# mkocabas/EpipolarPose

Measured on NVIDIA H100. Metric: multi-view samples/sec (4-view 256x256, bs32), higher is better.
Workload: dtype f16x3 (fp32 operands split into two fp16 planes, 3-pass error-compensated wgmma f16, f32 accumulate: fp32-grade results)

## Files before the change

### epipolarpose_b200/csrc/common.cuh

```cuda
#pragma once
#include <cuda_runtime.h>
#include <stdint.h>
#include <stdio.h>
#include <stdarg.h>
#include "../../include/epb.h"

void epb_set_error(const char* fmt, ...);

#define EPB_CHECK_ARG(cond)                                                   \
  do {                                                                        \
    if (!(cond)) {                                                            \
      epb_set_error("%s:%d: invalid argument: %s", __FILE__, __LINE__, #cond); \
      return EPB_EINVAL;                                                      \
    }                                                                         \
  } while (0)

#define EPB_CUDA(call)                                                        \
  do {                                                                        \
    cudaError_t e__ = (call);                                                 \
    if (e__ != cudaSuccess) {                                                 \
      epb_set_error("%s:%d: %s -> %s", __FILE__, __LINE__, #call,             \
                    cudaGetErrorString(e__));                                 \
      return EPB_ECUDA;                                                       \
    }                                                                         \
  } while (0)

#define EPB_LAUNCH_CHECK() EPB_CUDA(cudaGetLastError())

enum { EPB_WS_SOFTARGMAX = 1, EPB_WS_HMLOSS = 2, EPB_WS_BNCOEF = 3, EPB_WS_WPLANES = 4,
       EPB_WS_FPAIR = 5, EPB_WS_BNPART = 6, EPB_WS_SABWD = 7, EPB_WS_PATCHINV = 8, EPB_WS_KMEANS = 9 };
int epb_workspace(int kind, size_t bytes, cudaStream_t st, void** out);

static inline cudaStream_t as_stream(epb_stream_t s) { return (cudaStream_t)s; }

constexpr int kNumSMs = 132;

__device__ __forceinline__ float warp_sum(float v) {
#pragma unroll
  for (int o = 16; o > 0; o >>= 1) v += __shfl_xor_sync(0xffffffffu, v, o);
  return v;
}
__device__ __forceinline__ double warp_sum(double v) {
#pragma unroll
  for (int o = 16; o > 0; o >>= 1) v += __shfl_xor_sync(0xffffffffu, v, o);
  return v;
}
__device__ __forceinline__ float warp_max(float v) {
#pragma unroll
  for (int o = 16; o > 0; o >>= 1) v = fmaxf(v, __shfl_xor_sync(0xffffffffu, v, o));
  return v;
}
__device__ __forceinline__ float4 ldg_stream(const float4* p) {
  float4 r;
  asm volatile("ld.global.nc.L1::no_allocate.v4.f32 {%0,%1,%2,%3}, [%4];"
               : "=f"(r.x), "=f"(r.y), "=f"(r.z), "=f"(r.w) : "l"(p));
  return r;
}
```

### epipolarpose_b200/csrc/conv16.cu

```cuda
#include "split16_common.cuh"

namespace {

constexpr int BM = 128;
constexpr int kThreads16 = 384;
constexpr int kConsumers = 256;
constexpr int kStageBudget = 200 * 1024;
constexpr int kBoxBytes = 16 * 128;

struct Plan16 {
  epb_phase_grid grid;
  int Cout;
  int Wv, Hv;
  int T, CB;
  int n_tiles;
  int accumulate;
  int m_fastest;
  int splits;
  int koff[EPB_MAX_TAPS];
};

struct Maps16 {
  CUtensorMap a[4];
  CUtensorMap w;
  CUtensorMap out;
};

template <int BN>
struct Cfg16 {
  static constexpr int A_PLANE = BM * 128;
  static constexpr int B_PLANE = BN * 128;
  static constexpr int A_BYTES = 2 * A_PLANE;
  static constexpr int B_BYTES = 2 * B_PLANE;
  static constexpr int STAGE = A_BYTES + B_BYTES;
  static constexpr int S_ = kStageBudget / STAGE;
  static constexpr int S = S_ > 6 ? 6 : S_;
  static constexpr int BOX_BYTES = (kConsumers / 32) * kBoxBytes;
  static constexpr int STAT_BYTES = (kConsumers / 32) * 2 * BN * 4;
  static constexpr int SMEM =
      S * STAGE + BOX_BYTES + 1024  + 256  + STAT_BYTES;
  static_assert(SMEM <= 227 * 1024, "shared memory budget");
  static_assert(S >= 2, "ring too shallow");
};

template <int BN, bool SPLIT>
__global__ void __launch_bounds__(kThreads16, 1)
conv16_kernel(const __grid_constant__ Plan16 P, const __grid_constant__ Maps16 maps,
              const float* __restrict__ in_sc, const float* __restrict__ w_sc,
              const float* __restrict__ bias, double* __restrict__ stats) {
  using C = Cfg16<BN>;
  const epb_phase_grid& G = P.grid;
  constexpr int BOXES = C::S * C::STAGE;
  constexpr int CTRL = BOXES + C::BOX_BYTES;
  extern __shared__ uint8_t smem_raw[];
  tc::Ring<C::S, C::STAGE> ring(smem_raw, 0, CTRL, CTRL + 64);
  float* sstat = reinterpret_cast<float*>(ring.sm + CTRL + 256);

  const int warp = threadIdx.x >> 5, lane = threadIdx.x & 31;
  const int KB = P.T * P.CB;
  const int total_tiles = G.tiles * P.n_tiles;
  const int items = SPLIT ? total_tiles * P.splits : total_tiles;
  auto tile_of = [&](int item) { return SPLIT ? item % total_tiles : item; };
  auto kb_lo = [&](int s) { return SPLIT ? (int)((int64_t)s * KB / P.splits) : (s ? KB : 0); };
  auto nt_of = [&](int tile) { return P.m_fastest ? tile / G.tiles : tile % P.n_tiles; };
  auto mt_of = [&](int tile) { return P.m_fastest ? tile % G.tiles : tile / P.n_tiles; };

  if (threadIdx.x == 0) ring.init(1, kConsumers / 32);
  __syncthreads();

  if (warp < 4) {
    if (warp == 0 && lane == 0) {
      for (int v = 0; v < 4; ++v) tc::tma_prefetch_desc(&maps.a[v]);
      tc::tma_prefetch_desc(&maps.w);
      tc::tma_prefetch_desc(&maps.out);
      for (int item = blockIdx.x; item < items; item += gridDim.x) {
        const int tile = tile_of(item), s = SPLIT ? item / total_tiles : 0;
        const int nt = nt_of(tile);
        int w0, h0, n0;
        G.tile_origin(mt_of(tile), w0, h0, n0);
        const int kb0 = kb_lo(s), kb1 = kb_lo(s + 1);
        int t = kb0 / P.CB, cb = kb0 % P.CB;
        for (int kb = kb0; kb < kb1; ++kb) {
          tc::mbar_wait(ring.empty(ring.stage), ring.phase ^ 1);
          const uint32_t fb = ring.full(ring.stage);
          tc::mbar_arrive_expect_tx(fb, C::STAGE);
          const uint32_t a_dst = ring.stage_addr(ring.stage);
          const CUtensorMap* am = &maps.a[G.map[t]];
          const int cx = cb * 64, wx = w0 + G.dwq[t], hx = h0 + G.dhq[t];
          tc::tma_load_5d(a_dst, am, fb, cx, wx, hx, n0, 0);
          tc::tma_load_5d(a_dst + C::A_PLANE, am, fb, cx, wx, hx, n0, 1);
          const uint32_t b_dst = a_dst + C::A_BYTES;
          const int kx = P.koff[t] + cx, rx = nt * BN;
          tc::tma_load_3d(b_dst, &maps.w, fb, kx, rx, 0);
          tc::tma_load_3d(b_dst + C::B_PLANE, &maps.w, fb, kx, rx, 1);
          if (++cb == P.CB) { cb = 0; ++t; }
          ring.advance();
        }
      }
    }
    return;
  }

  const int wgc = (warp >> 2) - 1;
  const int ct = threadIdx.x - 128;
  float* wstat = sstat + (ct >> 5) * 2 * BN;
  const int lc = (lane & 3) * 2;
  const int rb = wgc * 64 + (warp & 3) * 16;
  const int ra = rb + (lane >> 2);
  uint8_t* box = ring.sm + BOXES + (ct >> 5) * kBoxBytes;
  const uint32_t box_addr = tc::smem_u32(box);
  auto chunk = [&](int jj) { return ((2 * jj + ((lane & 3) >> 1)) ^ (lane >> 2)) * 16 + (lane & 1) * 8; };
  const float alpha = in_sc[1] * w_sc[1];
  const int twh = G.tw * G.th;
  if (stats) {
    for (int c = ct; c < (kConsumers / 32) * 2 * BN; c += kConsumers) sstat[c] = 0.f;
    tc::named_sync(1, kConsumers);
  }

  float acc[BN / 2];
  int nt_prev = -1;
  for (int item = blockIdx.x; item < items; item += gridDim.x) {
    const int tile = tile_of(item), s = SPLIT ? item / total_tiles : 0;
    const int nt = nt_of(tile);
    if (stats && nt_prev >= 0 && nt != nt_prev)
      tc::stats_flush<BN, kConsumers / 32>(sstat, ct, nt_prev, P.Cout, stats);
    nt_prev = nt;
#pragma unroll
    for (int i = 0; i < BN / 2; ++i) acc[i] = 0.f;
    for (int kb = kb_lo(s), kb1 = kb_lo(s + 1); kb < kb1; ++kb)
      ring.consume(acc, [&](uint32_t st) {
        const uint32_t a_hi = st + wgc * 64 * 128, b_hi = st + C::A_BYTES;
#pragma unroll
        for (int kk = 0; kk < 4; ++kk)
          tc::mma3_f16<0, 0>(acc, tc::desc_kmajor_sw128(a_hi + kk * 32),
                             tc::desc_kmajor_sw128(a_hi + C::A_PLANE + kk * 32),
                             tc::desc_kmajor_sw128(b_hi + kk * 32),
                             tc::desc_kmajor_sw128(b_hi + C::B_PLANE + kk * 32));
      });
    ring.drain(acc);

    int w0, h0, n0;
    G.tile_origin(mt_of(tile), w0, h0, n0);
    bool srow[2];
#pragma unroll
    for (int h = 0; h < 2; ++h) {
      const int r = ra + 8 * h;
      const int w = w0 + r % G.tw, hh = h0 + (r / G.tw) % G.th, n = n0 + r / twh;
      srow[h] = w < G.Wp && hh < G.Hp && n < G.N;
    }
    const int bx = w0 + rb % G.tw, by = h0 + (rb / G.tw) % G.th, bz = n0 + rb / twh;
    const bool band = SPLIT || (bx < P.Wv && by < P.Hv && bz < G.N);
#pragma unroll
    for (int q = 0; q < BN / 32; ++q) {
      if (lane == 0) tc::tma_store_wait_read<0>();
      __syncwarp();
#pragma unroll
      float v[4][2][2];
#pragma unroll
      for (int jj = 0; jj < 4; ++jj) {
        const int col = nt * BN + 32 * q + 8 * jj + lc;
        float2 b = make_float2(0.f, 0.f);
        if (bias && col < P.Cout) b = *reinterpret_cast<const float2*>(bias + col);
#pragma unroll
        for (int h = 0; h < 2; ++h) {
          v[jj][h][0] = acc[16 * q + 4 * jj + 2 * h] * alpha + b.x;
          v[jj][h][1] = acc[16 * q + 4 * jj + 2 * h + 1] * alpha + b.y;
          *reinterpret_cast<float2*>(box + 128 * ((lane >> 2) + 8 * h) + chunk(jj)) =
              make_float2(v[jj][h][0], v[jj][h][1]);
        }
      }
      tc::fence_proxy_async();
      __syncwarp();
      const int c0 = nt * BN + 32 * q;
      if (lane == 0 && band && c0 < P.Cout) {
        if constexpr (SPLIT) tc::tma_store_4d(&maps.out, box_addr, c0, 0, (mt_of(tile) * BM + rb) / 16, s);
        else if (P.accumulate) tc::tma_reduce_add_4d(&maps.out, box_addr, c0, bx, by, bz);
        else tc::tma_store_4d(&maps.out, box_addr, c0, bx, by, bz);
        tc::tma_store_commit();
      }
      if (stats) {
#pragma unroll
        for (int jj = 0; jj < 4; ++jj) tc::stats_add<BN>(wstat, 32 * q + 8 * jj + lc, v[jj], srow);
      }
    }
  }
  if (stats && nt_prev >= 0) tc::stats_flush<BN, kConsumers / 32>(sstat, ct, nt_prev, P.Cout, stats);
  if (lane == 0) tc::tma_store_wait<0>();
}

struct Reduce16 {
  epb_phase_grid grid;
  int Cout, Wv, Hv, splits;
  int64_t sw, sh, sn;
};

__global__ void __launch_bounds__(256)
conv16_splitk_reduce(const __grid_constant__ Reduce16 R, const float* __restrict__ ws,
                     const float* __restrict__ bias, float* __restrict__ out,
                     double* __restrict__ stats) {
  __shared__ double red[2][8][128];
  const epb_phase_grid& G = R.grid;
  const int tx = threadIdx.x, ty = threadIdx.y;
  const int c = (blockIdx.x * 32 + tx) * 4;
  const bool cok = c < R.Cout;
  const int64_t M = (int64_t)G.N * G.Hp * G.Wp;
  const int64_t split_stride = (int64_t)G.tiles * BM * R.Cout;
  float b[4] = {0.f, 0.f, 0.f, 0.f};
  if (bias && cok)
    for (int e = 0; e < 4; ++e) b[e] = bias[c + e];
  double s1[4] = {0.0, 0.0, 0.0, 0.0}, s2[4] = {0.0, 0.0, 0.0, 0.0};
  if (cok) {
    for (int64_t m = (int64_t)blockIdx.y * 8 + ty; m < M; m += (int64_t)gridDim.y * 8) {
      const int w = (int)(m % G.Wp);
      const int64_t q = m / G.Wp;
      const int h = (int)(q % G.Hp), n = (int)(q / G.Hp);
      const int mt = w / G.tw + G.tiles_w * (h / G.th + G.tiles_h * (n / G.tn));
      const int r = w % G.tw + G.tw * (h % G.th + G.th * (n % G.tn));
      const float* src = ws + ((int64_t)mt * BM + r) * R.Cout + c;
      float4 v = *reinterpret_cast<const float4*>(src);
      for (int s = 1; s < R.splits; ++s) {
        const float4 u = *reinterpret_cast<const float4*>(src + s * split_stride);
        v.x += u.x; v.y += u.y; v.z += u.z; v.w += u.w;
      }
      v.x += b[0]; v.y += b[1]; v.z += b[2]; v.w += b[3];
      if (w < R.Wv && h < R.Hv)
        *reinterpret_cast<float4*>(out + n * R.sn + h * R.sh + w * R.sw + c) = v;
      const float a[4] = {v.x, v.y, v.z, v.w};
      for (int e = 0; e < 4; ++e) {
        s1[e] += a[e];
        s2[e] += (double)a[e] * a[e];
      }
    }
  }
  if (!stats) return;
  for (int e = 0; e < 4; ++e) {
    red[0][ty][tx * 4 + e] = s1[e];
    red[1][ty][tx * 4 + e] = s2[e];
  }
  __syncthreads();
  if (ty == 0 && cok)
    for (int e = 0; e < 4; ++e) {
      double t1 = 0.0, t2 = 0.0;
      for (int y = 0; y < 8; ++y) {
        t1 += red[0][y][tx * 4 + e];
        t2 += red[1][y][tx * 4 + e];
      }
      atomicAdd(stats + c + e, t1);
      atomicAdd(stats + R.Cout + c + e, t2);
    }
}

inline int conv16_bn(int Cout) { return Cout <= 64 ? 64 : 128; }

constexpr int kSplitMinKB = 4;
constexpr int kSplitLongKB = 16;

int conv16_run(const epb_conv_geom* g, const epb_half* in, const float* in_sc, const epb_half* w,
               const float* w_sc, const float* bias, float* out, double* stats, int splits,
               float* ws, epb_stream_t stream) {
  int rc = epb_conv_geom_check(g);
  if (rc) return rc;
  EPB_CHECK_ARG(in && in_sc && w && w_sc && out);
  EPB_CHECK_ARG(g->Cin % 64 == 0 && g->Cout % 4 == 0 && g->Cout >= 4);
  EPB_CHECK_ARG(g->is == 1 || g->is == 2);
  EPB_CHECK_ARG(!(stats && g->accumulate));
  EPB_CHECK_ARG((reinterpret_cast<uintptr_t>(in) & 127) == 0 && (reinterpret_cast<uintptr_t>(w) & 15) == 0);
  EPB_CHECK_ARG((reinterpret_cast<uintptr_t>(out) & 15) == 0 && (reinterpret_cast<uintptr_t>(bias) & 7) == 0);
  Plan16 P;
  Maps16 maps;
  memset(&maps, 0, sizeof(maps));
  bool dense;
  rc = epb_plan_phase_grid(g, in, BM, P.grid, maps.a, dense);
  if (rc) return rc;
  const int64_t Ho = dense ? 1 : g->Ho, Wo = dense ? P.grid.Wp : g->Wo, os = dense ? 1 : g->os;
  const int64_t ph = dense ? 0 : g->ph, pw = dense ? 0 : g->pw;
  P.Cout = g->Cout;
  P.Wv = dense ? P.grid.Wp : (g->Wo - g->pw + g->os - 1) / g->os;
  P.Hv = dense ? 1 : (g->Ho - g->ph + g->os - 1) / g->os;
  P.T = g->T; P.CB = g->Cin / 64; P.accumulate = g->accumulate;
  P.splits = splits;
  float* const view = out + (ph * Wo + pw) * g->Cout;
  if (splits == 1) {
    const int bw = P.grid.tw < 16 ? P.grid.tw : 16;
    const int bh = P.grid.th < 16 / bw ? P.grid.th : 16 / bw;
    const int64_t C4 = (int64_t)g->Cout * 4;
    const cuuint64_t dims[4] = {(cuuint64_t)g->Cout, (cuuint64_t)P.Wv, (cuuint64_t)P.Hv,
                                (cuuint64_t)P.grid.N};
    const cuuint64_t strides[3] = {(cuuint64_t)(os * C4), (cuuint64_t)(os * Wo * C4),
                                   (cuuint64_t)(Ho * Wo * C4)};
    const cuuint32_t box[4] = {32, (cuuint32_t)bw, (cuuint32_t)bh, (cuuint32_t)(16 / (bw * bh))};
    rc = epb_encode_map(&maps.out, CU_TENSOR_MAP_DATA_TYPE_FLOAT32, 4, view, dims, strides, box,
                        CU_TENSOR_MAP_L2_PROMOTION_NONE, "output");
    if (rc) return rc;
  } else {
    const int64_t C4 = (int64_t)g->Cout * 4;
    const cuuint64_t dims[4] = {(cuuint64_t)g->Cout, 16, (cuuint64_t)P.grid.tiles * (BM / 16),
                                (cuuint64_t)splits};
    const cuuint64_t strides[3] = {(cuuint64_t)C4, (cuuint64_t)(16 * C4),
                                   (cuuint64_t)((int64_t)P.grid.tiles * BM * C4)};
    const cuuint32_t box[4] = {32, 16, 1, 1};
    rc = epb_encode_map(&maps.out, CU_TENSOR_MAP_DATA_TYPE_FLOAT32, 4, ws, dims, strides, box,
                        CU_TENSOR_MAP_L2_PROMOTION_NONE, "split-K workspace");
    if (rc) return rc;
  }
  for (int t = 0; t < g->T; ++t) P.koff[t] = g->wt[t] * g->Cin;
  P.m_fastest = stats != nullptr;
  const int bn = conv16_bn(g->Cout);
  P.n_tiles = (g->Cout + bn - 1) / bn;
  const int64_t K = (int64_t)g->Tw * g->Cin;
  const cuuint64_t dims[3] = {(cuuint64_t)K, (cuuint64_t)g->Cout, 2};
  const cuuint64_t strides[2] = {(cuuint64_t)K * 2, (cuuint64_t)K * 2 * g->Cout};
  const cuuint32_t box[3] = {64, (cuuint32_t)bn, 1};
  rc = epb_encode_map(&maps.w, CU_TENSOR_MAP_DATA_TYPE_FLOAT16, 3, w, dims, strides, box,
                      CU_TENSOR_MAP_L2_PROMOTION_L2_256B, "weights");
  if (rc) return rc;
  const int64_t tiles = (int64_t)P.grid.tiles * P.n_tiles;
  cudaStream_t st = as_stream(stream);
  if (splits == 1) {
    const unsigned grid = (unsigned)(tiles < kNumSMs ? tiles : kNumSMs);
    if (bn == 64)
      return tc::launch<conv16_kernel<64, false>>(grid, kThreads16, Cfg16<64>::SMEM, st, P, maps,
                                                  in_sc, w_sc, bias, stats);
    return tc::launch<conv16_kernel<128, false>>(grid, kThreads16, Cfg16<128>::SMEM, st, P, maps,
                                                 in_sc, w_sc, bias, stats);
  }
  P.m_fastest = 0;
  const int64_t items = tiles * splits;
  const unsigned grid = (unsigned)(items < kNumSMs ? items : kNumSMs);
  const float* no_bias = nullptr;
  double* no_stats = nullptr;
  rc = bn == 64 ? tc::launch<conv16_kernel<64, true>>(grid, kThreads16, Cfg16<64>::SMEM, st, P, maps,
                                                      in_sc, w_sc, no_bias, no_stats)
                : tc::launch<conv16_kernel<128, true>>(grid, kThreads16, Cfg16<128>::SMEM, st, P,
                                                       maps, in_sc, w_sc, no_bias, no_stats);
  if (rc) return rc;
  Reduce16 R;
  R.grid = P.grid;
  R.Cout = g->Cout; R.Wv = P.Wv; R.Hv = P.Hv; R.splits = splits;
  R.sw = os * g->Cout; R.sh = os * Wo * g->Cout; R.sn = Ho * Wo * g->Cout;
  const int64_t M = (int64_t)P.grid.N * P.grid.Hp * P.grid.Wp;
  const unsigned gx = (unsigned)((g->Cout + 127) / 128);
  int64_t gy = (M + 7) / 8, cap = 4 * kNumSMs / gx + 1;
  if (gy > cap) gy = cap;
  conv16_splitk_reduce<<<dim3(gx, (unsigned)gy), dim3(32, 8), 0, st>>>(R, ws, bias, view, stats);
  EPB_LAUNCH_CHECK();
  return EPB_OK;
}

}

extern "C" __attribute__((visibility("default"))) int epb_conv16_fprop(
    const epb_conv_geom* g, const epb_half* in, const float* in_sc, const epb_half* w,
    const float* w_sc, const float* bias, float* out, double* stats, epb_stream_t stream) {
  return conv16_run(g, in, in_sc, w, w_sc, bias, out, stats, 1, nullptr, stream);
}

extern "C" __attribute__((visibility("default"))) int epb_conv16_splits(const epb_conv_geom* g,
                                                                          int* splits,
                                                                          long long* ws_floats) {
  int rc = epb_conv_geom_check(g);
  if (rc) return rc;
  EPB_CHECK_ARG(splits && ws_floats && g->Cin % 64 == 0 && g->Cout >= 4);
  epb_phase_grid G;
  bool dense;
  rc = epb_tile_phase_grid(g, BM, G, dense);
  if (rc) return rc;
  const int bn = conv16_bn(g->Cout);
  const int64_t tiles = (int64_t)G.tiles * ((g->Cout + bn - 1) / bn);
  const int64_t kb = (int64_t)g->T * (g->Cin / 64);
  int64_t s = kNumSMs / tiles;
  if (s > kb / kSplitMinKB) s = kb / kSplitMinKB;
  if (s < 4 && kb < kSplitLongKB * s) s = 1;
  if (s < 1) s = 1;
  *splits = (int)s;
  *ws_floats = s > 1 ? s * G.tiles * BM * g->Cout : 0;
  return EPB_OK;
}

extern "C" __attribute__((visibility("default"))) int epb_conv16_fprop_splitk(
    const epb_conv_geom* g, const epb_half* in, const float* in_sc, const epb_half* w,
    const float* w_sc, const float* bias, float* out, double* stats, int splits, float* ws,
    long long ws_floats, epb_stream_t stream) {
  int rc = epb_conv_geom_check(g);
  if (rc) return rc;
  EPB_CHECK_ARG(!g->accumulate);
  EPB_CHECK_ARG(g->Cin % 64 == 0 && splits >= 1 && splits <= g->T * (g->Cin / 64));
  if (splits > 1) {
    epb_phase_grid G;
    bool dense;
    rc = epb_tile_phase_grid(g, BM, G, dense);
    if (rc) return rc;
    EPB_CHECK_ARG(ws && (reinterpret_cast<uintptr_t>(ws) & 15) == 0);
    EPB_CHECK_ARG(ws_floats >= (long long)splits * G.tiles * BM * g->Cout);
  }
  return conv16_run(g, in, in_sc, w, w_sc, bias, out, stats, splits, ws, stream);
}
```

### epipolarpose_b200/csrc/split16.cu

```cuda
#include <cuda_fp16.h>
#include "common.cuh"

namespace {

constexpr int kThreads = 256;
constexpr float kHalfMax = 65504.f;

__device__ __forceinline__ void split2(float a, float b, float s, uint32_t& hi, uint32_t& lo) {
  a = fminf(fmaxf(a * s, -kHalfMax), kHalfMax);
  b = fminf(fmaxf(b * s, -kHalfMax), kHalfMax);
  const __half2 h = __floats2half2_rn(a, b);
  const float2 hf = __half22float2(h);
  const __half2 l = __floats2half2_rn(a - hf.x, b - hf.y);
  hi = *reinterpret_cast<const uint32_t*>(&h);
  lo = *reinterpret_cast<const uint32_t*>(&l);
}
__device__ __forceinline__ void split8(const float (&v)[8], float s, uint4& hi, uint4& lo) {
  split2(v[0], v[1], s, hi.x, lo.x);
  split2(v[2], v[3], s, hi.y, lo.y);
  split2(v[4], v[5], s, hi.z, lo.z);
  split2(v[6], v[7], s, hi.w, lo.w);
}
__device__ __forceinline__ float2 h2f(uint32_t u) {
  return __half22float2(*reinterpret_cast<const __half2*>(&u));
// ... 323 lines not shown
    sc[0] = s;
    sc[1] = 1.f / s;
  }
  for (int64_t i = (int64_t)blockIdx.x * kThreads + threadIdx.x; i < n4; i += (int64_t)gridDim.x * kThreads) {
    const float4 v = ldg_stream(src + i);
    uint2 hi, lo;
    split2(v.x, v.y, s, hi.x, lo.x);
    split2(v.z, v.w, s, hi.y, lo.y);
    dst[i] = hi;
    dst[n4 + i] = lo;
  }
}


struct RowMap {
  int C4, tpr, rpi, chunks;
};
inline RowMap make_rowmap(int C) {
  RowMap r;
  r.C4 = C / 4;
  r.tpr = r.C4 < kThreads ? r.C4 : kThreads;
  r.rpi = kThreads / r.tpr;
  if (r.rpi < 1) r.rpi = 1;
  r.chunks = (r.C4 + r.tpr - 1) / r.tpr;
  return r;
}

__device__ __forceinline__ float4 mask4(float4 dy, float4 xv, const uint2* mask_hi, int64_t i,
                                        float4 s, float4 b, int relu) {
  if (mask_hi) {
    const uint2 m = mask_hi[i];
    return make_float4((m.x & 0x7fffu) ? dy.x : 0.f, (m.x & 0x7fff0000u) ? dy.y : 0.f,
                       (m.y & 0x7fffu) ? dy.z : 0.f, (m.y & 0x7fff0000u) ? dy.w : 0.f);
  }
  if (relu) {
    return make_float4(fmaf(xv.x, s.x, b.x) > 0.f ? dy.x : 0.f, fmaf(xv.y, s.y, b.y) > 0.f ? dy.y : 0.f,
                       fmaf(xv.z, s.z, b.z) > 0.f ? dy.z : 0.f, fmaf(xv.w, s.w, b.w) > 0.f ? dy.w : 0.f);
  }
  return dy;
}

template <int MASK>
__device__ __forceinline__ uint2 load_mask(const uint2* mask, int64_t i) {
  if (MASK == 1) return __ldg(mask + i);
  const unsigned byte = __ldg(reinterpret_cast<const uint8_t*>(mask) + (i >> 1));
  return make_uint2((i & 1) ? (byte >> 4) : (byte & 15u), 0u);
}

template <int MASK>
__global__ void __launch_bounds__(kThreads, 3)
bn_bwd_partial_kernel(const float4* __restrict__ dy, const float4* __restrict__ x,
                      const uint2* __restrict__ mask_hi, const float4* __restrict__ scale,
                      const float4* __restrict__ shift, const float4* __restrict__ mean,
                      const float4* __restrict__ invstd, int relu, int64_t M, int C, RowMap rm,
                      float* __restrict__ parts, uint32_t* __restrict__ bound_bits) {
  if (bound_bits && blockIdx.x == 0 && blockIdx.y == 0 && threadIdx.x == 0) *bound_bits = 0u;
  const int slot = threadIdx.x / rm.tpr, tin = threadIdx.x % rm.tpr;
  const int c4 = blockIdx.y * rm.tpr + tin;
  const bool active = (c4 < rm.C4) && (slot < rm.rpi);
  const int64_t nblk = (M + rm.rpi - 1) / rm.rpi;
  float4 acc[4] = {{0, 0, 0, 0}, {0, 0, 0, 0}, {0, 0, 0, 0}, {0, 0, 0, 0}};
  if (active) {
    const float4 mu = mean[c4], is = invstd[c4];
    float4 s = make_float4(0, 0, 0, 0), b = s;
    if (!MASK) { s = scale[c4]; b = shift[c4]; }
    auto fold = [&](float4 dv, float4 xv, uint2 mk) {
      float4 g;
      if (MASK == 1) {
        g = make_float4((mk.x & 0x7fffu) ? dv.x : 0.f, (mk.x & 0x7fff0000u) ? dv.y : 0.f,
                        (mk.y & 0x7fffu) ? dv.z : 0.f, (mk.y & 0x7fff0000u) ? dv.w : 0.f);
      } else if (MASK == 2) {
        g = make_float4((mk.x & 1u) ? dv.x : 0.f, (mk.x & 2u) ? dv.y : 0.f,
                        (mk.x & 4u) ? dv.z : 0.f, (mk.x & 8u) ? dv.w : 0.f);
      } else {
        g = mask4(dv, xv, nullptr, 0, s, b, relu);
      }
      const float4 xh = make_float4((xv.x - mu.x) * is.x, (xv.y - mu.y) * is.y,
                                    (xv.z - mu.z) * is.z, (xv.w - mu.w) * is.w);
      acc[0].x += g.x; acc[0].y += g.y; acc[0].z += g.z; acc[0].w += g.w;
      acc[1].x += g.x * xh.x; acc[1].y += g.y * xh.y; acc[1].z += g.z * xh.z; acc[1].w += g.w * xh.w;
      acc[2].x = fmaxf(acc[2].x, fabsf(g.x)); acc[2].y = fmaxf(acc[2].y, fabsf(g.y));
      acc[2].z = fmaxf(acc[2].z, fabsf(g.z)); acc[2].w = fmaxf(acc[2].w, fabsf(g.w));
      acc[3].x = fmaxf(acc[3].x, fabsf(xh.x)); acc[3].y = fmaxf(acc[3].y, fabsf(xh.y));
      acc[3].z = fmaxf(acc[3].z, fabsf(xh.z)); acc[3].w = fmaxf(acc[3].w, fabsf(xh.w));
    };
    int64_t blk = blockIdx.x;
    const int64_t step = gridDim.x;
    for (; blk + 3 * step < nblk; blk += 4 * step) {
      float4 xv[4], dv[4];
      uint2 mk[4];
      bool ok[4];
#pragma unroll
      for (int u = 0; u < 4; ++u) {
        const int64_t r = (blk + u * step) * rm.rpi + slot;
        ok[u] = r < M;
        mk[u] = make_uint2(0u, 0u);
        if (ok[u]) {
          const int64_t i = r * rm.C4 + c4;
          xv[u] = ldg_stream(x + i);
          dv[u] = ldg_stream(dy + i);
          if (MASK) mk[u] = load_mask<MASK>(mask_hi, i);
        }
      }
#pragma unroll
      for (int u = 0; u < 4; ++u)
        if (ok[u]) fold(dv[u], xv[u], mk[u]);
    }
    for (; blk < nblk; blk += step) {
      const int64_t r = blk * rm.rpi + slot;
      if (r >= M) break;
      const int64_t i = r * rm.C4 + c4;
      const float4 xv = ldg_stream(x + i);
      const float4 dv = ldg_stream(dy + i);
      fold(dv, xv, MASK ? load_mask<MASK>(mask_hi, i) : make_uint2(0u, 0u));
    }
  }
  __shared__ float4 sh[4][kThreads];
#pragma unroll
  for (int v = 0; v < 4; ++v) sh[v][threadIdx.x] = acc[v];
  __syncthreads();
  if (slot == 0 && active) {
    const int64_t W = gridDim.x;
#pragma unroll
    for (int v = 0; v < 4; ++v) {
      float4 t = sh[v][tin];
      for (int q = 1; q < rm.rpi; ++q) {
        const float4 u = sh[v][q * rm.tpr + tin];
        if (v < 2) { t.x += u.x; t.y += u.y; t.z += u.z; t.w += u.w; }
        else { t.x = fmaxf(t.x, u.x); t.y = fmaxf(t.y, u.y); t.z = fmaxf(t.z, u.z); t.w = fmaxf(t.w, u.w); }
      }
      *reinterpret_cast<float4*>(parts + ((int64_t)v * W + blockIdx.x) * C + c4 * 4) = t;
    }
  }
}

__global__ void __launch_bounds__(256)
bn_bwd_combine_kernel(const float* __restrict__ parts, int W, double M, int C,
                      double* __restrict__ sums, float* __restrict__ maxes, float* __restrict__ coef,
                      const float* __restrict__ gamma, const float* __restrict__ invstd,
                      float* __restrict__ dgamma, float* __restrict__ dbeta,
                      uint32_t* __restrict__ bound_bits) {
  const int ch = threadIdx.x & 7, g = threadIdx.x >> 3;
  const int c = blockIdx.x * 8 + ch;
  double a0 = 0, a1 = 0;
  float m0 = 0.f, m1 = 0.f;
  if (c < C) {
    const float* p0 = parts + c;
    const int64_t plane = (int64_t)W * C;
    for (int w0 = g; w0 < W; w0 += 32 * 8) {
      float v[4][8];
#pragma unroll
      for (int u = 0; u < 8; ++u) {
        const int w = w0 + 32 * u;
        const int64_t o = (int64_t)(w < W ? w : 0) * C;
#pragma unroll
        for (int k = 0; k < 4; ++k) v[k][u] = (w < W) ? __ldg(p0 + k * plane + o) : 0.f;
      }
#pragma unroll
      for (int u = 0; u < 8; ++u) {
        a0 += (double)v[0][u];
        a1 += (double)v[1][u];
        m0 = fmaxf(m0, v[2][u]);
        m1 = fmaxf(m1, v[3][u]);
      }
    }
  }
  __shared__ double sa[2][32][8];
  __shared__ float sm[2][32][8];
  sa[0][g][ch] = a0; sa[1][g][ch] = a1;
  sm[0][g][ch] = m0; sm[1][g][ch] = m1;
  __syncthreads();
#pragma unroll
  for (int half = 16; half > 0; half >>= 1) {
    if (g < half) {
      sa[0][g][ch] += sa[0][g + half][ch];
      sa[1][g][ch] += sa[1][g + half][ch];
      sm[0][g][ch] = fmaxf(sm[0][g][ch], sm[0][g + half][ch]);
      sm[1][g][ch] = fmaxf(sm[1][g][ch], sm[1][g + half][ch]);
    }
    __syncthreads();
  }
  if (g != 0) return;
  a0 = sa[0][0][ch]; a1 = sa[1][0][ch];
  m0 = sm[0][0][ch]; m1 = sm[1][0][ch];
  float bound = 0.f;
  if (c < C) {
    if (!coef) {
      sums[c] += a0;
      sums[C + c] += a1;
      maxes[c] = fmaxf(maxes[c], m0);
      maxes[C + c] = fmaxf(maxes[C + c], m1);
    } else {
      const float k0 = (gamma ? gamma[c] : 1.f) * invstd[c];
      const float k1 = (float)(a0 / M), k2 = (float)(a1 / M);
      coef[c] = k1;
      coef[C + c] = k2;
      if (dgamma) dgamma[c] = (float)a1;
      if (dbeta) dbeta[c] = (float)a0;
      bound = fabsf(k0) * (m0 + fabsf(k1) + m1 * fabsf(k2));
    }
  }
  if (coef) {
    for (int o = 4; o > 0; o >>= 1) bound = fmaxf(bound, __shfl_xor_sync(0xffu, bound, o));
    if (ch == 0) atomicMax(bound_bits, __float_as_uint(bound));
  }
}

__global__ void __launch_bounds__(1024)
bn_bwd_coef_split_kernel(const double* __restrict__ sums, float* __restrict__ maxes, double M, int C,
                         const float* __restrict__ gamma, const float* __restrict__ invstd,
                         float* __restrict__ dz_sc, float* __restrict__ dgamma,
                         float* __restrict__ dbeta) {
  float bound = 0.f;
  for (int c = threadIdx.x; c < C; c += blockDim.x) {
    const double sg = sums[c], sgx = sums[C + c];
    const float k0 = (gamma ? gamma[c] : 1.f) * invstd[c];
    const float k1 = (float)(sg / M), k2 = (float)(sgx / M);
    const float mg = maxes[c], mx = maxes[C + c];
    bound = fmaxf(bound, fabsf(k0) * (mg + fabsf(k1) + mx * fabsf(k2)));
    maxes[c] = k1;
    maxes[C + c] = k2;
    if (dgamma) dgamma[c] = (float)sgx;
    if (dbeta) dbeta[c] = (float)sg;
  }
  bound = warp_max(bound);
  __shared__ float sm[32];
  if ((threadIdx.x & 31) == 0) sm[threadIdx.x >> 5] = bound;
  __syncthreads();
  if (threadIdx.x == 0) {
    for (int w = 1; w < (int)(blockDim.x >> 5); ++w) bound = fmaxf(bound, sm[w]);
    const float s = pow2_scale(bound);
    dz_sc[0] = s;
    dz_sc[1] = 1.f / s;
  }
}

__global__ void __launch_bounds__(kThreads)
bn_bwd_apply_split_kernel(const float4* dy , const float4* __restrict__ x,
                          const uint2* __restrict__ mask_hi, const float4* __restrict__ scale,
                          const float4* __restrict__ shift, const float4* __restrict__ mean,
                          const float4* __restrict__ invstd, const float4* __restrict__ gamma,
                          int relu, const float4* __restrict__ k1v, const float4* __restrict__ k2v,
                          uint2* __restrict__ dz, float* __restrict__ dz_sc,
                          const float* __restrict__ bound, float4* dy_masked, int64_t total4, int C4,
                          int mask_bits) {
  const float s = bound ? pow2_scale(*bound) : dz_sc[0];
  if (bound && blockIdx.x == 0 && threadIdx.x == 0) {
    dz_sc[0] = s;
    dz_sc[1] = 1.f / s;
  }
  const int64_t stride = (int64_t)gridDim.x * kThreads;
  for (int64_t i0 = (int64_t)blockIdx.x * kThreads + threadIdx.x; i0 < total4; i0 += 2 * stride) {
    const int64_t idx[2] = {i0, i0 + stride};
    float4 xv[2], dv[2];
    uint2 mk[2];
#pragma unroll
    for (int u = 0; u < 2; ++u) {
      if (idx[u] < total4) {
        xv[u] = ldg_stream(x + idx[u]);
        dv[u] = __ldcs(dy + idx[u]);
        if (mask_hi) mk[u] = mask_bits ? load_mask<2>(mask_hi, idx[u]) : mask_hi[idx[u]];
      }
    }
#pragma unroll
    for (int u = 0; u < 2; ++u) {
      const int64_t i = idx[u];
      if (i >= total4) break;
      const int c4 = (int)(i % C4);
      float4 g = dv[u];
      if (mask_hi && mask_bits) {
        g = make_float4((mk[u].x & 1u) ? g.x : 0.f, (mk[u].x & 2u) ? g.y : 0.f,
                        (mk[u].x & 4u) ? g.z : 0.f, (mk[u].x & 8u) ? g.w : 0.f);
      } else if (mask_hi) {
        g = make_float4((mk[u].x & 0x7fffu) ? g.x : 0.f, (mk[u].x & 0x7fff0000u) ? g.y : 0.f,
                        (mk[u].y & 0x7fffu) ? g.z : 0.f, (mk[u].y & 0x7fff0000u) ? g.w : 0.f);
      } else {
        g = mask4(g, xv[u], nullptr, i, scale[c4], shift[c4], relu);
      }
      const float4 mu = mean[c4], is = invstd[c4], b = k1v[c4], c = k2v[c4];
      float4 a = is;
      if (gamma) {
        const float4 ga = gamma[c4];
        a.x *= ga.x; a.y *= ga.y; a.z *= ga.z; a.w *= ga.w;
      }
      float4 o;
      o.x = a.x * (g.x - b.x - (xv[u].x - mu.x) * is.x * c.x);
      o.y = a.y * (g.y - b.y - (xv[u].y - mu.y) * is.y * c.y);
      o.z = a.z * (g.z - b.z - (xv[u].z - mu.z) * is.z * c.z);
      o.w = a.w * (g.w - b.w - (xv[u].w - mu.w) * is.w * c.w);
      uint2 hi, lo;
      split2(o.x, o.y, s, hi.x, lo.x);
      split2(o.z, o.w, s, hi.y, lo.y);
      dz[i] = hi;
      dz[total4 + i] = lo;
      if (dy_masked) dy_masked[i] = g;
    }
  }
}

__device__ __forceinline__ double channel_bound(double s1, double s2, double sc, double sh, double M) {
  const double mean = s1 / M, q = s2 / M;
  double var = q - mean * mean;
  if (var < 0) var = 0;
  const double ku = (16.0 + ceil(M / (16.0 * kNumSMs))) * 0x1p-24;
  return fabs(sc * mean + sh) + fabs(sc) * (sqrt(M * (var + 4.0 * ku * q)) + ku * sqrt(q));
}

__device__ __forceinline__ float group_bound(const double* stats, const float* scale,
                                             const float* shift, double M, int C) {
  float b = 0.f;
  for (int c = threadIdx.x; c < C; c += blockDim.x)
    b = fmaxf(b, (float)channel_bound(stats[c], stats[C + c], scale[c], shift[c], M));
  return b;
}

__device__ __forceinline__ void publish_act_scale(float b1, float b2, const float* res_sc, float* sc) {
  float bound = (b1 + b2) * 1.001f + (res_sc ? res_sc[2] : 0.f);
  if (!isfinite(bound)) bound = 3.0e38f;
  float s = 1.f;
  if (bound > 0.f) {
    int e;
    frexpf(bound, &e);
    int k = 15 - e;
    k = k < -100 ? -100 : (k > 100 ? 100 : k);
    s = ldexpf(1.f, k);
  }
  sc[0] = s;
  sc[1] = 1.f / s;
  sc[2] = bound;
  sc[3] = 0.f;
}

__global__ void __launch_bounds__(1024)
act_scale_kernel(const double* __restrict__ stats, const float* __restrict__ scale,
                 const float* __restrict__ shift, double M, int C,
                 const double* __restrict__ stats2, const float* __restrict__ scale2,
                 const float* __restrict__ shift2, const float* __restrict__ res_sc,
                 float* __restrict__ sc) {
  float b1 = group_bound(stats, scale, shift, M, C);
  float b2 = stats2 ? group_bound(stats2, scale2, shift2, M, C) : 0.f;
  b1 = warp_max(b1);
  b2 = warp_max(b2);
  __shared__ float sm[2][32];
  if ((threadIdx.x & 31) == 0) { sm[0][threadIdx.x >> 5] = b1; sm[1][threadIdx.x >> 5] = b2; }
  __syncthreads();
  if (threadIdx.x == 0) {
    for (int w = 1; w < (int)(blockDim.x >> 5); ++w) { b1 = fmaxf(b1, sm[0][w]); b2 = fmaxf(b2, sm[1][w]); }
    publish_act_scale(b1, b2, res_sc, sc);
  }
}

__global__ void __launch_bounds__(1024)
bn_finalize_scale_kernel(const double* __restrict__ stats, double M, int C,
                         const float* __restrict__ gamma, const float* __restrict__ beta, float eps,
                         float momentum, float* __restrict__ running_mean,
                         float* __restrict__ running_var, float* __restrict__ scale,
                         float* __restrict__ shift, float* __restrict__ mean_out,
                         float* __restrict__ invstd_out, const double* __restrict__ stats2,
                         const float* __restrict__ scale2, const float* __restrict__ shift2,
                         const float* __restrict__ res_sc, float* __restrict__ sc) {
  float b1 = 0.f;
  for (int c = threadIdx.x; c < C; c += blockDim.x) {
    const double mean = stats[c] / M;
    double var = stats[C + c] / M - mean * mean;
    if (var < 0) var = 0;
    const double invstd = 1.0 / sqrt(var + (double)eps);
    const float g = gamma ? gamma[c] : 1.f, b = beta ? beta[c] : 0.f;
    const float scf = (float)(g * invstd), shf = (float)(b - mean * g * invstd);
    scale[c] = scf;
    shift[c] = shf;
    if (mean_out) mean_out[c] = (float)mean;
    if (invstd_out) invstd_out[c] = (float)invstd;
    if (running_mean) {
      const double unbiased = var * (M / (M > 1.0 ? (M - 1.0) : 1.0));
      running_mean[c] = (float)((1.0 - momentum) * running_mean[c] + momentum * mean);
      running_var[c] = (float)((1.0 - momentum) * running_var[c] + momentum * unbiased);
    }
    b1 = fmaxf(b1, (float)channel_bound(stats[c], stats[C + c], scf, shf, M));
  }
  float b2 = stats2 ? group_bound(stats2, scale2, shift2, M, C) : 0.f;
  b1 = warp_max(b1);
  b2 = warp_max(b2);
  __shared__ float sm[2][32];
  if ((threadIdx.x & 31) == 0) { sm[0][threadIdx.x >> 5] = b1; sm[1][threadIdx.x >> 5] = b2; }
  __syncthreads();
  if (threadIdx.x == 0) {
    for (int w = 1; w < (int)(blockDim.x >> 5); ++w) { b1 = fmaxf(b1, sm[0][w]); b2 = fmaxf(b2, sm[1][w]); }
    publish_act_scale(b1, b2, res_sc, sc);
  }
}

__global__ void __launch_bounds__(1024)
softargmax_bwd_bound_kernel(const float* __restrict__ lse, const float* __restrict__ dcoords, int NJ,
                            float* __restrict__ sc) {
  float b = 0.f;
  for (int i = threadIdx.x; i < NJ; i += blockDim.x)
    b = fmaxf(b, lse[i * 2 + 1] * (fabsf(dcoords[i * 3]) + fabsf(dcoords[i * 3 + 1]) + fabsf(dcoords[i * 3 + 2])));
  b = warp_max(b);
  __shared__ float sm[32];
  if ((threadIdx.x & 31) == 0) sm[threadIdx.x >> 5] = b;
  __syncthreads();
  if (threadIdx.x == 0) {
    for (int w = 1; w < (int)(blockDim.x >> 5); ++w) b = fmaxf(b, sm[w]);
    const float s = pow2_scale(b);
    sc[0] = s;
    sc[1] = 1.f / s;
  }
}

__global__ void softargmax_bwd_split_kernel(const float* __restrict__ logits, int J, int D, int H, int W,
                                            int S, int ppi, const float* __restrict__ coords,
                                            const float* __restrict__ lse,
                                            const float* __restrict__ dcoords,
                                            const float* __restrict__ sc, uint2* __restrict__ planes,
                                            int64_t total4, float* __restrict__ parts) {
  extern __shared__ float4 shq[];
  const int n = blockIdx.y, sp = blockIdx.x;
  const int C4 = (J * D) >> 2;
  const int HW = H * W;
  const int per = (HW + S - 1) / S;
  const int pbeg = sp * per, pend = min(HW, pbeg + per);
  const int c4 = threadIdx.x % C4, sub = threadIdx.x / C4;
  const int D4 = D >> 2;
  const int j = c4 / D4;
  const float z0 = (float)((c4 % D4) << 2);
  const int nj = n * J + j;
  const float m = lse[nj * 2], inv = lse[nj * 2 + 1];
  const float gx = dcoords[nj * 3] / W, gy = dcoords[nj * 3 + 1] / H, gz = dcoords[nj * 3 + 2] / D;
  const float sbar = gx * (coords[nj * 3] + 0.5f) * W + gy * (coords[nj * 3 + 1] + 0.5f) * H +
                     gz * (coords[nj * 3 + 2] + 0.5f) * D;
  const float s = sc[0];
  const int64_t img = (int64_t)n * HW * C4 + c4;
  const float4* base = reinterpret_cast<const float4*>(logits) + img;
  float4 acc = make_float4(0.f, 0.f, 0.f, 0.f);
  int pix = pbeg + sub;
  int y = pix / W, x = pix - y * W;
  for (; pix < pend; pix += ppi) {
    const float4 v = ldg_stream(base + (int64_t)pix * C4);
    const float s0 = gx * x + gy * y + gz * z0 - sbar;
    float4 o;
    o.x = __expf(v.x - m) * inv * (s0);
    o.y = __expf(v.y - m) * inv * (s0 + gz);
    o.z = __expf(v.z - m) * inv * (s0 + 2.f * gz);
    o.w = __expf(v.w - m) * inv * (s0 + 3.f * gz);
    uint2 hi, lo;
    split2(o.x, o.y, s, hi.x, lo.x);
    split2(o.z, o.w, s, hi.y, lo.y);
    const int64_t i = img + (int64_t)pix * C4;
    planes[i] = hi;
    planes[total4 + i] = lo;
    acc.x += o.x; acc.y += o.y; acc.z += o.z; acc.w += o.w;
    x += ppi;
    while (x >= W) { x -= W; ++y; }
  }
  shq[threadIdx.x] = acc;
  __syncthreads();
  if (sub == 0) {
    for (int q = 1; q < ppi; ++q) {
      const float4 t = shq[q * C4 + c4];
      acc.x += t.x; acc.y += t.y; acc.z += t.z; acc.w += t.w;
    }
    reinterpret_cast<float4*>(parts)[((int64_t)n * S + sp) * C4 + c4] = acc;
  }
}

__global__ void __launch_bounds__(256)
colsum_parts_kernel(const float* __restrict__ parts, int rows, int C, float* __restrict__ out) {
  const int ch = threadIdx.x & 7, g = threadIdx.x >> 3;
  const int c = blockIdx.x * 8 + ch;
  double a = 0;
  if (c < C) {
    for (int r0 = g; r0 < rows; r0 += 32 * 16) {
      float v[16];
#pragma unroll
      for (int u = 0; u < 16; ++u) {
        const int r = r0 + 32 * u;
        v[u] = (r < rows) ? __ldg(parts + (int64_t)r * C + c) : 0.f;
      }
#pragma unroll
      for (int u = 0; u < 16; ++u) a += (double)v[u];
    }
  }
  __shared__ double sa[32][8];
  sa[g][ch] = a;
  __syncthreads();
#pragma unroll
  for (int half = 16; half > 0; half >>= 1) {
    if (g < half) sa[g][ch] += sa[g + half][ch];
    __syncthreads();
  }
  if (g == 0 && c < C) out[c] = (float)sa[0][ch];
}

__global__ void avgpool_split_kernel(const __half* __restrict__ x, const float* __restrict__ x_sc,
                                     float* __restrict__ y, int N, int HW, int C) {
  const int n = blockIdx.y, c = blockIdx.x * blockDim.x + threadIdx.x;
  if (c >= C) return;
  const int64_t plane = (int64_t)N * HW * C;
  float acc = 0.f;
  for (int p = 0; p < HW; ++p) {
    const int64_t i = ((int64_t)n * HW + p) * C + c;
    acc += __half2float(x[i]) + __half2float(x[plane + i]);
  }
  y[(int64_t)n * C + c] = acc * x_sc[1] / (float)HW;
}

}

#define EPB_API extern "C" __attribute__((visibility("default")))

EPB_API int epb_bn_act_split(const float* x, const float* scale, const float* shift, const float* r,
                             const float* rscale, const float* rshift, const epb_half* r_split,
                             const float* r_sc, int relu, int64_t M, int C, epb_half* y,
                             const float* y_sc, uint8_t* mask_bits, epb_stream_t stream) {
  EPB_CHECK_ARG(x && y && y_sc && M > 0 && C > 0 && C % 8 == 0);
  EPB_CHECK_ARG((scale == nullptr) == (shift == nullptr));
  EPB_CHECK_ARG((rscale == nullptr) == (rshift == nullptr));
  EPB_CHECK_ARG(!(r && r_split) && ((r_split == nullptr) == (r_sc == nullptr)));
  EPB_CHECK_ARG(!rscale || r);
  const int64_t total8 = M * (C / 8);
  bn_act_split_kernel<<<ew_blocks(total8), kThreads, 0, as_stream(stream)>>>(
      x, scale, shift, r, rscale, rshift, reinterpret_cast<const uint4*>(r_split), r_sc, relu, total8,
      C / 8, reinterpret_cast<uint4*>(y), y_sc, mask_bits);
  EPB_LAUNCH_CHECK();
  return EPB_OK;
}

EPB_API int epb_bn_relu_maxpool_split(const float* x, const float* scale, const float* shift,
                                      epb_half* y, const float* y_sc, uint8_t* argidx, int N, int H,
                                      int W, int C, epb_stream_t stream) {
  EPB_CHECK_ARG(x && scale && shift && y && y_sc && N > 0 && H > 0 && W > 0 && C > 0 && C % 8 == 0);
  const int Ho = (H + 2 - 3) / 2 + 1, Wo = (W + 2 - 3) / 2 + 1;
  const int64_t total = (int64_t)N * Ho * Wo * (C / 8);
  bn_relu_maxpool_split_kernel<<<ew_blocks(total), kThreads, 0, as_stream(stream)>>>(
      x, scale, shift, reinterpret_cast<uint4*>(y), y_sc, reinterpret_cast<uint2*>(argidx), N, H, W,
      C / 8);
  EPB_LAUNCH_CHECK();
  return EPB_OK;
}

EPB_API int epb_im2col_split(const float* img_nchw, epb_half* col, const float* col_sc, int N, int C,
                             int Hi, int Wi, int kh, int kw, int stride, int pad, int Ho, int Wo,
                             int Kpad, epb_stream_t stream) {
  EPB_CHECK_ARG(img_nchw && col && col_sc && N > 0 && C > 0 && Kpad % 8 == 0 && Kpad >= kh * kw * C);
  const int64_t total = (int64_t)N * Ho * Wo * (Kpad / 8);
  EPB_CHECK_ARG(Kpad <= 4096);
  {
    const int tw = stride * (kSeg - 1) + kw, segs = (Wo + kSeg - 1) / kSeg;
    const size_t smem = ((size_t)Kpad + (size_t)C * kh * tw) * sizeof(int);
    const int64_t ctas = (int64_t)N * Ho * segs;
    if (smem <= 48 * 1024 && ctas < (1LL << 31)) {
      im2col_split_tiled_kernel<<<(unsigned)ctas, kThreads, smem, as_stream(stream)>>>(
          img_nchw, reinterpret_cast<uint4*>(col), col_sc, N, C, Hi, Wi, kh, kw, stride, pad, Ho, Wo, Kpad,
          segs, tw);
      EPB_LAUNCH_CHECK();
      return EPB_OK;
    }
  }
  im2col_split_kernel<<<ew_blocks(total), kThreads, 2 * Kpad * sizeof(int), as_stream(stream)>>>(
      img_nchw, reinterpret_cast<uint4*>(col), col_sc, N, C, Hi, Wi, kh, kw, stride, pad, Ho, Wo, Kpad);
  EPB_LAUNCH_CHECK();
  return EPB_OK;
}

EPB_API int epb_split16_batch(const epb_split_job* jobs, int njobs, long long total_blocks,
                              uint32_t* amax_ws, epb_stream_t stream) {
  EPB_CHECK_ARG(jobs && amax_ws && njobs > 0 && total_blocks > 0 && total_blocks < (1LL << 31));
  cudaStream_t st = as_stream(stream);
  EPB_CUDA(cudaMemsetAsync(amax_ws, 0, sizeof(uint32_t) * njobs, st));
  split_amax_kernel<<<(unsigned)total_blocks, kThreads, 0, st>>>(jobs, njobs, amax_ws);
  EPB_LAUNCH_CHECK();
  split_apply_kernel<<<(unsigned)total_blocks, kThreads, 0, st>>>(jobs, njobs, amax_ws);
  EPB_LAUNCH_CHECK();
  return EPB_OK;
}

static int bn_bwd_workers(const RowMap& rm, int64_t M) {
  const int64_t nblk = (M + rm.rpi - 1) / rm.rpi;
  int64_t workers = (nblk + 3) / 4;
  const int64_t cap = (int64_t)kNumSMs * 3 / rm.chunks > 1 ? (int64_t)kNumSMs * 3 / rm.chunks : 1;
  if (workers > cap) workers = cap;
  return (int)(workers < 1 ? 1 : workers);
}
static int bn_bwd_scratch(int W, int C, cudaStream_t st, float** parts, float** coef, uint32_t** bound) {
  void* p = nullptr;
  const size_t nparts = (size_t)4 * W * C;
  size_t bytes = (nparts + 2 * (size_t)C + 4) * sizeof(float);
  const size_t usual = ((size_t)4 * 3 * kNumSMs * 2048 + 2 * 2048 + 4) * sizeof(float);
  if (bytes < usual) bytes = usual;
  int rc = epb_workspace(EPB_WS_BNPART, bytes, st, &p);
  if (rc) return rc;
  *parts = static_cast<float*>(p);
  *coef = *parts + nparts;
  *bound = reinterpret_cast<uint32_t*>(*coef + 2 * (size_t)C);
  return EPB_OK;
}

static void launch_bn_bwd_partial(const float* dy, const float* x, const epb_half* mask_hi,
                                  const float* scale, const float* shift, const float* mean,
                                  const float* invstd, int relu, int64_t M, int C, const RowMap& rm,
                                  int W, float* parts, uint32_t* bound, cudaStream_t st,
                                  int mask_kind = 1) {
  auto k = mask_kind == 2 ? bn_bwd_partial_kernel<2> : (mask_hi ? bn_bwd_partial_kernel<1> : bn_bwd_partial_kernel<0>);
  k<<<dim3(W, rm.chunks), kThreads, 0, st>>>(
      reinterpret_cast<const float4*>(dy), reinterpret_cast<const float4*>(x),
      reinterpret_cast<const uint2*>(mask_hi), reinterpret_cast<const float4*>(scale),
      reinterpret_cast<const float4*>(shift), reinterpret_cast<const float4*>(mean),
// ... 165 lines not shown
```

Baseline: 487.1.

## Pin each conv16 CTA to one output-channel tile when accumulating BN stats

When batch-norm statistics are requested, each CTA is now bound to a single N tile (blockIdx % n_tiles) and walks M tiles in strided runs, so the per-CTA shared-memory stat buffer is flushed only at run boundaries instead of whenever the N tile changes. The grid is rounded to a multiple of n_tiles, and the error bound used for activation scaling is updated to match the new per-run accumulation length. This is meant to cut the number of double-precision atomic stat flushes, at the cost of possible load imbalance and less weight-tile sharing across CTAs in L2.

Result: faster. 494.8 (median of 6 runs) (+1.6%).

```diff
diff --git a/epipolarpose_b200/csrc/common.cuh b/epipolarpose_b200/csrc/common.cuh
--- a/epipolarpose_b200/csrc/common.cuh
+++ b/epipolarpose_b200/csrc/common.cuh
@@ -35,6 +35,11 @@
 
 constexpr int kNumSMs = 132;
 
+constexpr int kConv16StatsStride = kNumSMs;
+__host__ __device__ constexpr int64_t conv16_stats_run(int64_t tiles) {
+  return (tiles + kConv16StatsStride - 1) / kConv16StatsStride;
+}
+
 __device__ __forceinline__ float warp_sum(float v) {
 #pragma unroll
   for (int o = 16; o > 0; o >>= 1) v += __shfl_xor_sync(0xffffffffu, v, o);
diff --git a/epipolarpose_b200/csrc/conv16.cu b/epipolarpose_b200/csrc/conv16.cu
--- a/epipolarpose_b200/csrc/conv16.cu
+++ b/epipolarpose_b200/csrc/conv16.cu
@@ -15,7 +15,6 @@
   int T, CB;
   int n_tiles;
   int accumulate;
-  int m_fastest;
   int splits;
   int koff[EPB_MAX_TAPS];
 };
@@ -43,7 +42,7 @@
   static_assert(S >= 2, "ring too shallow");
 };
 
-template <int BN, bool SPLIT>
+template <int BN, bool SPLIT, bool OWN>
 __global__ void __launch_bounds__(kThreads16, 1)
 conv16_kernel(const __grid_constant__ Plan16 P, const __grid_constant__ Maps16 maps,
               const float* __restrict__ in_sc, const float* __restrict__ w_sc,
@@ -60,10 +59,32 @@
   const int KB = P.T * P.CB;
   const int total_tiles = G.tiles * P.n_tiles;
   const int items = SPLIT ? total_tiles * P.splits : total_tiles;
-  auto tile_of = [&](int item) { return SPLIT ? item % total_tiles : item; };
+  static_assert(!(SPLIT && OWN), "the split-K kernel sums no statistics");
+  constexpr bool own = OWN;
+  const int run0 = own ? blockIdx.x / P.n_tiles : 0;
+  const int runs = G.tiles < kConv16StatsStride ? G.tiles : kConv16StatsStride;
+  auto valid = [&](int run, int pos) { return own ? run < runs : pos < items; };
+  auto next = [&](int& run, int& pos) {
+    if (!own) {
+      pos += gridDim.x;
+    } else if ((pos += kConv16StatsStride) >= G.tiles) {
+      run += gridDim.x / P.n_tiles;
+      pos = run;
+    }
+  };
+  auto decode = [&](int pos, int& mt, int& nt, int& s) {
+    if (own) {
+      mt = pos;
+      nt = blockIdx.x % P.n_tiles;
+      s = 0;
+      return;
+    }
+    const int tile = SPLIT ? pos % total_tiles : pos;
+    s = SPLIT ? pos / total_tiles : 0;
+    nt = tile % P.n_tiles;
+    mt = tile / P.n_tiles;
+  };
   auto kb_lo = [&](int s) { return SPLIT ? (int)((int64_t)s * KB / P.splits) : (s ? KB : 0); };
-  auto nt_of = [&](int tile) { return P.m_fastest ? tile / G.tiles : tile % P.n_tiles; };
-  auto mt_of = [&](int tile) { return P.m_fastest ? tile % G.tiles : tile / P.n_tiles; };
 
   if (threadIdx.x == 0) ring.init(1, kConsumers / 32);
   __syncthreads();
@@ -73,11 +94,11 @@
       for (int v = 0; v < 4; ++v) tc::tma_prefetch_desc(&maps.a[v]);
       tc::tma_prefetch_desc(&maps.w);
       tc::tma_prefetch_desc(&maps.out);
-      for (int item = blockIdx.x; item < items; item += gridDim.x) {
-        const int tile = tile_of(item), s = SPLIT ? item / total_tiles : 0;
-        const int nt = nt_of(tile);
+      for (int run = run0, pos = own ? run0 : blockIdx.x; valid(run, pos); next(run, pos)) {
+        int mt, nt, s;
+        decode(pos, mt, nt, s);
         int w0, h0, n0;
-        G.tile_origin(mt_of(tile), w0, h0, n0);
+        G.tile_origin(mt, w0, h0, n0);
         const int kb0 = kb_lo(s), kb1 = kb_lo(s + 1);
         int t = kb0 / P.CB, cb = kb0 % P.CB;
         for (int kb = kb0; kb < kb1; ++kb) {
@@ -118,13 +139,11 @@
   }
 
   float acc[BN / 2];
-  int nt_prev = -1;
-  for (int item = blockIdx.x; item < items; item += gridDim.x) {
-    const int tile = tile_of(item), s = SPLIT ? item / total_tiles : 0;
-    const int nt = nt_of(tile);
-    if (stats && nt_prev >= 0 && nt != nt_prev)
-      tc::stats_flush<BN, kConsumers / 32>(sstat, ct, nt_prev, P.Cout, stats);
-    nt_prev = nt;
+  for (int run = run0, pos = own ? run0 : blockIdx.x; valid(run, pos); next(run, pos)) {
+    int mt, nt, s;
+    decode(pos, mt, nt, s);
+    if (stats && pos == run && run != run0)
+      tc::stats_flush<BN, kConsumers / 32>(sstat, ct, nt, P.Cout, stats);
 #pragma unroll
     for (int i = 0; i < BN / 2; ++i) acc[i] = 0.f;
     for (int kb = kb_lo(s), kb1 = kb_lo(s + 1); kb < kb1; ++kb)
@@ -140,7 +159,7 @@
     ring.drain(acc);
 
     int w0, h0, n0;
-    G.tile_origin(mt_of(tile), w0, h0, n0);
+    G.tile_origin(mt, w0, h0, n0);
     bool srow[2];
 #pragma unroll
     for (int h = 0; h < 2; ++h) {
@@ -173,7 +192,7 @@
       __syncwarp();
       const int c0 = nt * BN + 32 * q;
       if (lane == 0 && band && c0 < P.Cout) {
-        if constexpr (SPLIT) tc::tma_store_4d(&maps.out, box_addr, c0, 0, (mt_of(tile) * BM + rb) / 16, s);
+        if constexpr (SPLIT) tc::tma_store_4d(&maps.out, box_addr, c0, 0, (mt * BM + rb) / 16, s);
         else if (P.accumulate) tc::tma_reduce_add_4d(&maps.out, box_addr, c0, bx, by, bz);
         else tc::tma_store_4d(&maps.out, box_addr, c0, bx, by, bz);
         tc::tma_store_commit();
@@ -184,7 +203,7 @@
       }
     }
   }
-  if (stats && nt_prev >= 0) tc::stats_flush<BN, kConsumers / 32>(sstat, ct, nt_prev, P.Cout, stats);
+  if (stats) tc::stats_flush<BN, kConsumers / 32>(sstat, ct, blockIdx.x % P.n_tiles, P.Cout, stats);
   if (lane == 0) tc::tma_store_wait<0>();
 }
 
@@ -304,7 +323,6 @@
     if (rc) return rc;
   }
   for (int t = 0; t < g->T; ++t) P.koff[t] = g->wt[t] * g->Cin;
-  P.m_fastest = stats != nullptr;
   const int bn = conv16_bn(g->Cout);
   P.n_tiles = (g->Cout + bn - 1) / bn;
   const int64_t K = (int64_t)g->Tw * g->Cin;
@@ -317,22 +335,30 @@
   const int64_t tiles = (int64_t)P.grid.tiles * P.n_tiles;
   cudaStream_t st = as_stream(stream);
   if (splits == 1) {
-    const unsigned grid = (unsigned)(tiles < kNumSMs ? tiles : kNumSMs);
+    unsigned grid = (unsigned)(tiles < kNumSMs ? tiles : kNumSMs);
+    if (stats) {
+      const int g_nt = (int)grid / P.n_tiles;
+      grid = (unsigned)((g_nt > 1 ? g_nt : 1) * P.n_tiles);
+      if (bn == 64)
+        return tc::launch<conv16_kernel<64, false, true>>(grid, kThreads16, Cfg16<64>::SMEM, st, P,
+                                                          maps, in_sc, w_sc, bias, stats);
+      return tc::launch<conv16_kernel<128, false, true>>(grid, kThreads16, Cfg16<128>::SMEM, st, P,
+                                                         maps, in_sc, w_sc, bias, stats);
+    }
     if (bn == 64)
-      return tc::launch<conv16_kernel<64, false>>(grid, kThreads16, Cfg16<64>::SMEM, st, P, maps,
-                                                  in_sc, w_sc, bias, stats);
-    return tc::launch<conv16_kernel<128, false>>(grid, kThreads16, Cfg16<128>::SMEM, st, P, maps,
-                                                 in_sc, w_sc, bias, stats);
-  }
-  P.m_fastest = 0;
+      return tc::launch<conv16_kernel<64, false, false>>(grid, kThreads16, Cfg16<64>::SMEM, st, P, maps,
+                                                         in_sc, w_sc, bias, stats);
+    return tc::launch<conv16_kernel<128, false, false>>(grid, kThreads16, Cfg16<128>::SMEM, st, P, maps,
+                                                        in_sc, w_sc, bias, stats);
+  }
   const int64_t items = tiles * splits;
   const unsigned grid = (unsigned)(items < kNumSMs ? items : kNumSMs);
   const float* no_bias = nullptr;
   double* no_stats = nullptr;
-  rc = bn == 64 ? tc::launch<conv16_kernel<64, true>>(grid, kThreads16, Cfg16<64>::SMEM, st, P, maps,
-                                                      in_sc, w_sc, no_bias, no_stats)
-                : tc::launch<conv16_kernel<128, true>>(grid, kThreads16, Cfg16<128>::SMEM, st, P,
-                                                       maps, in_sc, w_sc, no_bias, no_stats);
+  rc = bn == 64 ? tc::launch<conv16_kernel<64, true, false>>(grid, kThreads16, Cfg16<64>::SMEM, st, P,
+                                                             maps, in_sc, w_sc, no_bias, no_stats)
+                : tc::launch<conv16_kernel<128, true, false>>(grid, kThreads16, Cfg16<128>::SMEM, st, P,
+                                                              maps, in_sc, w_sc, no_bias, no_stats);
   if (rc) return rc;
   Reduce16 R;
   R.grid = P.grid;
diff --git a/epipolarpose_b200/csrc/split16.cu b/epipolarpose_b200/csrc/split16.cu
--- a/epipolarpose_b200/csrc/split16.cu
+++ b/epipolarpose_b200/csrc/split16.cu
@@ -649,7 +649,7 @@
   const double mean = s1 / M, q = s2 / M;
   double var = q - mean * mean;
   if (var < 0) var = 0;
-  const double ku = (16.0 + ceil(M / (16.0 * kNumSMs))) * 0x1p-24;
+  const double ku = (16.0 + (double)conv16_stats_run((int64_t)ceil(M / 16.0))) * 0x1p-24;
   return fabs(sc * mean + sh) + fabs(sc) * (sqrt(M * (var + 4.0 * ku * q)) + ku * sqrt(q));
 }
 
```
